# jianhengLiu/VINS-RGBD-FAST

Measured on AMD Instinct MI355X. Metric: VIO frames/sec (640x480, 150 feats, 10-KF window), higher is better.
Workload: dtype f64; 1 GPU; BASELINE configs[2]: 128 independent synthetic 640x480 RGB-D + 200 Hz IMU sequences per MI355X, 150 features, 10-keyframe window; sequences_per_gpu=128, tracker_lag=1, parallelism=sequences sharded per GPU, no data-path collective

## Files before the change

include/vio_abi.h:

```cpp
#ifndef VIO_ABI_H
#define VIO_ABI_H
#include <stddef.h>
#include <stdint.h>
#ifdef __cplusplus
extern "C" {
#endif

enum {
    VIO_OK = 0,
    VIO_NEED_IMU = 1,
    VIO_REBOOTED = 2,
    VIO_EINVAL = -1,
    VIO_EDEVICE = -2,
    VIO_ECAPACITY = -3
};

typedef struct vio_config {
    int32_t width, height;
    int32_t max_cnt, min_dist;
    int32_t grid_rows, grid_cols;
    int32_t window_size;
    int32_t max_landmarks;
    int32_t fix_depth;
    int32_t estimate_extrinsic;
// ... 121 lines not shown
int vio_get_camera(vio_batch *h, int seq, vio_camera *out);
#define VIO_SNAPSHOT_MAGIC 0x0050414E534F4956ULL
#define VIO_SNAPSHOT_FORMAT 1
typedef struct vio_snapshot_shape {
    int32_t width, height, max_cnt, min_dist, grid_rows, grid_cols, window_size, max_landmarks, fix_depth, estimate_extrinsic, estimate_td,
        max_iterations, ransac_max_iters, lk_max_level, dynamic_init, use_imu, reference_quirks, marg_exact, equalize;
    int32_t imu_capacity;
    int32_t hist_cap;
    int32_t pyramid_levels;
    int32_t reserved[2];
    double focal_length, f_threshold, depth_min, depth_max, min_parallax_px, init_depth;
} vio_snapshot_shape;
typedef struct vio_snapshot_header {
    uint64_t magic;
    uint32_t format_version;
    uint32_t abi_version;
    int64_t total_bytes;
    int64_t device_bytes;
    int64_t host_bytes;
    int64_t frames_processed;
    double last_stamp;
    int32_t tracker_lag;
    int32_t solver_flag;
    vio_snapshot_shape shape;
} vio_snapshot_header;
int vio_shape_key(const vio_config *cfg, int imu_capacity, vio_snapshot_shape *out);
int vio_snapshot_info(const void *blob, int64_t bytes, vio_snapshot_header *out);
int64_t vio_snapshot_bytes(vio_batch *h, int seq);
int vio_save_seqs(vio_batch *h, int n, const int32_t *seqs, void *dst, const int64_t *offsets, const int64_t *caps, int64_t *bytes_out);
int vio_load_seqs(vio_batch *h, int n, const int32_t *seqs, const void *src, const int64_t *offsets, const int64_t *bytes);
int64_t vio_debug_save_seq_naive(vio_batch *h, int seq, void *dst, int64_t cap);
int64_t vio_debug_snapshot_staging_bytes(vio_batch *h);
int vio_debug_snapshot_layout(vio_batch *h, int i, char *name64, int32_t *kind, int64_t *bytes_per_seq, int64_t *blob_offset);
int vio_get_tracks(vio_batch *h, int seq, int cap, int32_t *ids, int32_t *track_cnt, float *cur_pts_xy, float *cur_un_pts_xy,
                   float *pts_velocity_xy);
int vio_get_landmarks(vio_batch *h, int seq, int cap, double *out);
int vio_get_landmarks_ex(vio_batch *h, int seq, int cap, double *out12);
int vio_get_prior(vio_batch *h, int seq, double *J_nxn, double *r_n, double *x0, uint8_t *present);

int vio_get_timings(vio_batch *h, int cap, double *out_ms);
int vio_profile_begin(vio_batch *h, int max_steps);
int vio_profile_end(vio_batch *h, int cap, double *out_ms);
void *vio_get_stream(vio_batch *h);

int vio_stage_pyr_down(const uint8_t *src, int w, int h, uint8_t *dst);
int vio_stage_clahe(const uint8_t *src, int w, int h, uint8_t *dst);
int vio_stage_fast_roi(const uint8_t *img, int W, int H, int rx, int ry, int rw, int rh, int cap, float *out_xys);
int vio_lk_effective_level(int width, int height, int lk_max_level);
int vio_stage_lk(const uint8_t *prev, const uint8_t *next, int w, int h, int max_level, int n, const float *prev_pts,
                 float *next_pts_inout, uint8_t *status);
int vio_stage_ransac(const vio_config *cfg, int n, const float *p1, const float *p2, uint8_t *status);
int vio_stage_relative_r(int n, const double *corres6, double *R9);
int vio_stage_relative_r_detail(int n, const double *corres6, double *R9, int *detail8);
int vio_stage_imu_factor(const vio_config *cfg, int n, const double *dt, const double *acc, const double *gyr,
                         const double *acc0, const double *gyr0, const double *ba, const double *bg, const double *pose_i,
                         const double *sb_i, const double *pose_j, const double *sb_j, double *preint_out, double *r15,
                         double *J480);
int vio_stage_projection(const vio_config *cfg, const double *pose_i, const double *pose_j, const double *ex, double inv_dep,
                         double td, const double *obs_i, const double *obs_j, int use_td, double *r2, double *J46);
int vio_stage_projection_residual(const vio_config *cfg, const double *pose_i, const double *pose_j, const double *ex, double inv_dep,
                                  double td, const double *obs_i, const double *obs_j, int use_td, double *r2, double *J46);
int vio_stage_pnp(int n, const double *obj, const double *img, double *rvec3, double *tvec3);
int vio_stage_pnp_trace(int n, const double *obj, const double *img, double *rvec3, double *tvec3, int *trace4);
int vio_stage_host_pnp_trace(int n, const double *obj, const double *img, double *rvec3, double *tvec3, int *trace4);
int vio_stage_rodrigues(int mode, int n, const double *in, double *out);
int vio_stage_host_rodrigues(int mode, int n, const double *in, double *out);
// ... 36 lines not shown
```

vins-rgbd-fast_amd/__init__.py:

```python
import ctypes as C
import os
import subprocess

import numpy as np

_HERE = os.path.dirname(os.path.abspath(__file__))
_LIB_PATH = os.path.join(_HERE, "libvio_hip.so")

VIO_OK, VIO_NEED_IMU, VIO_REBOOTED = 0, 1, 2
VIO_EINVAL, VIO_EDEVICE, VIO_ECAPACITY = -1, -2, -3


class VioError(RuntimeError):
    pass


class Config(C.Structure):
    _fields_ = [(n, C.c_int32) for n in (
        "width", "height", "max_cnt", "min_dist", "grid_rows", "grid_cols", "window_size", "max_landmarks", "fix_depth",
        "estimate_extrinsic", "estimate_td", "max_iterations", "ransac_max_iters", "lk_max_level", "dynamic_init", "use_imu", "reference_quirks",
        "marg_exact", "equalize")] + \
        [(n, C.c_double) for n in ("fx", "fy", "cx", "cy", "k1", "k2", "p1", "p2", "focal_length", "f_threshold", "depth_min",
                                   "depth_max", "acc_n", "acc_w", "gyr_n", "gyr_w", "g_norm")] + \
        [("ric", C.c_double * 9), ("tic", C.c_double * 3)] + \
# ... 565 lines not shown
    def process_obs(self, seq, ids, obs, depth, stamp):
        ids = np.ascontiguousarray(ids, np.int32).reshape(-1)
        obs = np.ascontiguousarray(obs, np.float64).reshape(-1, 7)
        depth = np.ascontiguousarray(depth, np.uint16)
        self._keep3 = (ids, obs, depth)
        self._chk(self.L.vio_process_obs(self.h, seq, len(ids), ids.ctypes.data, obs.ctypes.data, depth.ctypes.data, float(stamp)),
                  "vio_process_obs")

    def process_obs_batch(self, n_obs, ids, obs, depth, stamps, on_device=False):
        n_obs = np.ascontiguousarray(n_obs, np.int32).reshape(self.S)
        ids = np.ascontiguousarray(ids, np.int32).reshape(self.S, -1)
        cap = ids.shape[1]
        obs = np.ascontiguousarray(obs, np.float64).reshape(self.S, cap, 7)
        stamps = np.ascontiguousarray(stamps, np.float64).reshape(self.S)
        self._keep3 = (n_obs, ids, obs, depth, stamps)
        self._chk(self.L.vio_process_obs_batch(self.h, n_obs.ctypes.data, ids.ctypes.data, obs.ctypes.data, cap, _ptr(depth),
                                               stamps.ctypes.data, 1 if on_device else 0), "vio_process_obs_batch")

    def packaged(self, seq=0, cap=2048):
        ids, obs = np.zeros(cap, np.int32), np.zeros((cap, 7))
        n = self._chk(self.L.vio_get_packaged(self.h, seq, cap, ids.ctypes.data, obs.ctypes.data), "vio_get_packaged")
        return ids[:n].copy(), obs[:n].copy()

    def solver_kind(self):
        self.L.vio_get_solver_kind.argtypes = [C.c_void_p]
        return self.L.vio_get_solver_kind(self.h)

    def bound_stats(self, seq=0):
        o = np.zeros(4, np.int64)
        self.L.vio_get_bound_stats.argtypes = [C.c_void_p, C.c_int, C.c_void_p]
        self._chk(self.L.vio_get_bound_stats(self.h, int(seq), o.ctypes.data), "vio_get_bound_stats")
        return tuple(int(x) for x in o)

    def ex_calibration(self, seq=0, history=False):
        o = np.zeros(16, np.float64)
        hist = np.zeros((2048 if history else 0, 12), np.float64)
        n = self._chk(self.L.vio_get_ex_calibration(self.h, int(seq), o.ctypes.data, hist.shape[0], hist.ctypes.data if history else None),
                      "vio_get_ex_calibration")
        out = dict(state=int(o[0]), pairs=int(o[1]), success_frame=int(o[2]), ric=o[3:12].reshape(3, 3).copy(), sv=o[12:16].copy())
        if history:
            out["history"] = hist[:min(n, hist.shape[0])].reshape(-1, 3, 4).copy()
        return out

    def marg_certificate(self, seq=0):
        o = np.zeros(2, np.int32)
        self.L.vio_get_marg_certificate.argtypes = [C.c_void_p, C.c_int, C.c_void_p]
        self._chk(self.L.vio_get_marg_certificate(self.h, int(seq), o.ctypes.data), "vio_get_marg_certificate")
        return int(o[0]), bool(o[1])

    def capacity(self):
        c = np.zeros(3, np.int32)
        self._chk(self.L.vio_get_capacity(self.h, c.ctypes.data), "vio_get_capacity")
        return dict(tracks=int(c[0]), landmarks=int(c[1]), imu=int(c[2]))

    def reset_seq(self, seq):
        self._chk(self.L.vio_reset_seq(self.h, seq), "vio_reset_seq")

    def reset_tracker_seq(self, seq):
        self._chk(self.L.vio_reset_tracker_seq(self.h, seq), "vio_reset_tracker_seq")

    def sync(self):
        self._chk(self.L.vio_sync(self.h), "vio_sync")

    def reset(self):
        self._chk(self.L.vio_reset(self.h), "vio_reset")

# ... 178 lines not shown
```

vins-rgbd-fast_amd/csrc/abi_query.hip:

```cpp
#include "vio_handle.h"

namespace vio_internal {

std::string calibration_check(const vio_calibration &k) {
    const struct { const char *name; const double *v; int n; } fin[] = {
        {"fx", &k.fx, 1}, {"fy", &k.fy, 1}, {"cx", &k.cx, 1}, {"cy", &k.cy, 1}, {"k1", &k.k1, 1}, {"k2", &k.k2, 1}, {"p1", &k.p1, 1},
        {"p2", &k.p2, 1}, {"ric", k.ric, 9}, {"tic", k.tic, 3}, {"td", &k.td, 1}, {"tr", &k.tr, 1}, {"acc_n", &k.acc_n, 1},
        {"acc_w", &k.acc_w, 1}, {"gyr_n", &k.gyr_n, 1}, {"gyr_w", &k.gyr_w, 1}, {"g_norm", &k.g_norm, 1}};
    for (const auto &f : fin)
        for (int i = 0; i < f.n; i++)
            if (!std::isfinite(f.v[i])) return std::string(f.name) + " is not finite";
    const struct { const char *name; double v; } pos[] = {
        {"fx", k.fx}, {"fy", k.fy}, {"acc_n", k.acc_n}, {"acc_w", k.acc_w}, {"gyr_n", k.gyr_n}, {"gyr_w", k.gyr_w}, {"g_norm", k.g_norm}};
    for (const auto &f : pos)
        if (!(f.v > 0)) return std::string(f.name) + " must be > 0";
    if (!(k.tr >= 0)) return "tr must be >= 0";
    {
        double err = 0;
        for (int i = 0; i < 3; i++)
            for (int j = 0; j < 3; j++) {
                double d = (i == j) ? -1.0 : 0.0;
                for (int q = 0; q < 3; q++) d += k.ric[3 * i + q] * k.ric[3 * j + q];
                err = std::max(err, std::fabs(d));
            }
// ... 433 lines not shown
    int n = h->hc.NPRIOR, W = h->hc.W;
    if (J || r) {
        be_prior_factor_kernel<<<1, 512, h->lds_factor, h->stream>>>(h->B, seq);
        HIPCHK(hipGetLastError());
        HIPCHK(hipStreamSynchronize(h->stream));
    }
    if (J) HIPCHK(hipMemcpy(J, h->B.prior_J + (size_t)seq * n * n, sizeof(double) * n * n, hipMemcpyDeviceToHost));
    if (r) HIPCHK(hipMemcpy(r, h->B.prior_rf + (size_t)seq * n, sizeof(double) * n, hipMemcpyDeviceToHost));
    if (x0) HIPCHK(hipMemcpy(x0, h->B.prior_x0 + (size_t)seq * (W * 7 + 17), sizeof(double) * (W * 7 + 17), hipMemcpyDeviceToHost));
    if (present) for (int k = 0; k < W + 3; k++) present[k] = (uint8_t)be.prior_present[k];
    return n;
}

int vio_get_timings(vio_batch *h, int cap, double *out_ms) {
    VIO_ENTER(h, VIO_NO_SEQ, false);
    if (!out_ms || cap < 3) return VIO_EINVAL;
    if (!h->timing_valid) return 0;
    VIO_TRY(sync_all(h));
    float a = 0, b = 0;
    HIPCHK(hipEventElapsedTime(&a, h->ev[0], h->ev[1]));
    HIPCHK(hipEventElapsedTime(&b, h->ev[1], h->ev[2]));
    out_ms[0] = a; out_ms[1] = b; out_ms[2] = a + b;
    return 3;
}

int vio_debug_seq(vio_batch *h, int seq, int *out16) {
    VIO_ENTER(h, seq, true);
    static thread_local BeSeq be;
    HIPCHK(hipMemcpy(&be, h->B.be + seq, sizeof(BeSeq), hipMemcpyDeviceToHost));
    for (int k = 0; k < 16; k++) out16[k] = be.dbg[k];
    return VIO_OK;
}

int vio_debug_phases(vio_batch *h, float *out128, int reset) {
    VIO_ENTER(h, VIO_NO_SEQ, true);
    if (out128) HIPCHK(hipMemcpy(out128, h->B.timings, 128 * sizeof(float), hipMemcpyDeviceToHost));
    if (reset) HIPCHK(hipMemset(h->B.timings, 0, 128 * sizeof(float)));
    return VIO_OK;
}

int vio_debug_fe_ticks(vio_batch *h, float *out) {
    VIO_ENTER(h, VIO_NO_SEQ, true);
    if (!out) return VIO_EINVAL;
    HIPCHK(hipMemcpy(out, h->B.fe_ticks, (size_t)h->S * 4 * sizeof(float), hipMemcpyDeviceToHost));
    return VIO_OK;
}

int vio_profile_begin(vio_batch *h, int max_steps) {
    VIO_ENTER(h, VIO_NO_SEQ, false);
    if (max_steps < 1) return VIO_EINVAL;
    size_t need = (size_t)max_steps * VIO_NEV;
    while (h->pev.size() < need) {
        hipEvent_t e;
        VIO_TRY(new_event(h, &e, hipEventDefault));
        h->pev.push_back(e);
    }
    h->prof_steps = max_steps;
    h->prof_cur = 0;
    h->prof_fe_only = false;
    return VIO_OK;
}
int vio_profile_end(vio_batch *h, int cap, double *out_ms) {
    VIO_ENTER(h, VIO_NO_SEQ, true);
    if (!out_ms || cap < VIO_NK) return VIO_EINVAL;
    int n = h->prof_cur < 0 ? 0 : (h->prof_cur < h->prof_steps ? h->prof_cur : h->prof_steps);
    static const int e0[VIO_NK] = {0, 1, 2, 3, 4, 5, 6, 8, 9, 10}, e1[VIO_NK] = {1, 2, 3, 4, 5, 6, 7, 9, 10, 11};
// ... 14 lines not shown
```

vins-rgbd-fast_amd/csrc/be_kernels.hip:

```cpp
#include <hip/hip_runtime.h>
#include "kernels.h"
#include "be_factors.h"

using namespace dm;

#if VIO_TIMERS
#define PH_INIT long long ph_t0 = (s == 0 && threadIdx.x == 0) ? VIO_CLOCK() : 0
#define PH(k) do { if (s == 0 && threadIdx.x == 0) { long long n_ = VIO_CLOCK(); B.timings[k] += (float)(n_ - ph_t0); ph_t0 = n_; } } while (0)
#else
#define PH_INIT do {} while (0)
#define PH(k) do {} while (0)
#endif

namespace {

struct Ctx {
    float *timings;
    const DevCfg *C;
    int s, W, P, LW, NL, NLs, NPR;
    BeSeq *be;
    FeSeq *fe;
    const vio_calibration *K;
    PreInt *pre;
    int *lm_id, *lm_start, *lm_nobs, *lm_est, *lm_solve, *lm_dyn, *lm_order, *lm_free, *lm_tmp, *lm_pidx, *lm_aidx, *lm_relo;
// ... 497 lines not shown
                } else { dep = rsum / rn; ef = 0; }
            } else { dep = vsum / vn; ef = 1; }
            if (dep < 0.1) { dep = cfg.init_depth; ef = 0; }
            c.lm_depth[slot] = dep;
            c.lm_est[slot] = ef;
        }
}

__device__ void repropagate_window(Ctx &c, PreWork &pw) {
    const int t = threadIdx.x, nt = blockDim.x, W = c.W;
    BeSeq &be = *c.be;
    const vio_config &cfg = c.C->c;
    for (int j = 0; j <= W; j++) {
            PreInt &p = c.pre[be.pre_idx[j]];
            if (!p.valid) continue;
            if (t == 0) {
                int nb = p.n_buf;
                v3 la = ld3(p.lin_acc), lg = ld3(p.lin_gyr);
                p.sum_dt = 0;
                st3(p.acc0, la); st3(p.gyr0, lg);
                p.dp[0] = p.dp[1] = p.dp[2] = 0; p.dv[0] = p.dv[1] = p.dv[2] = 0;
                p.dq[0] = 1; p.dq[1] = p.dq[2] = p.dq[3] = 0;
                p.lin_ba[0] = p.lin_ba[1] = p.lin_ba[2] = 0;
                st3(p.lin_bg, ld3(be.Bgs[j]));
                p.n_buf = nb;
            }
            for (int i = t; i < 225; i += nt) { pw.J[i] = ((i / 15) == (i % 15)) ? 1.0 : 0.0; pw.Pm[i] = 0; }
            __syncthreads();
            for (int q = 0; q < p.n_buf; q++) preint_propagate(p, pw, *c.K, p.dt_buf[q], ld3(p.acc_buf[q]), ld3(p.gyr_buf[q]));
            preint_store(p, pw);
        }
}

template <bool EXCALIB>
__global__ __launch_bounds__(256) void be_ingest_kernel(Batch B, const uint16_t *depth_base, size_t depth_stride, IngestSrc src) {
    const int s = blockIdx.x + B.s0, t = threadIdx.x, nt = blockDim.x;
    Ctx c = make_ctx(B, s);
    const DevCfg &C = *B.cfg;
    const vio_config &cfg = C.c;
    const vio_calibration &K = *c.K;
    BeSeq &be = *c.be;
    FeSeq &fe = *c.fe;
    const int W = c.W;
    __shared__ int sh_i[8];
    __shared__ double sh_d[8];
    __shared__ int scratch[2 * 256 + 8];
    __shared__ double sred[256];
    __shared__ PreWork pw;
    PH_INIT;
    const bool ext = src.ids != nullptr;
    const int ext_n = ext ? src.n_obs[s] : 0;
    const double in_stamp = ext ? src.stamps[s] : fe.cur_time;
    if (t == 0) {
        for (int k = 0; k < 3; k++) be.track_Bg[k] = be.latest_Bg[k];
        be.track_td = be.td;
        be.imu_count_ingest = be.imu_count;
        be.do_solve = 0; be.do_marg = 0; be.processed = 0; be.rebooted = 0; be.init_frame = 0; be.dyn_failed = 0;
        be.status_code = (!ext && fe.n_forw == -2) ? VIO_NEED_IMU : VIO_OK;
        be.cur_stamp = in_stamp;
        be.overflow = 0;
        if (be.imu_count - be.imu_head > C.NIMU) { be.imu_head = be.imu_count - C.NIMU; be.overflow |= 16; }
    }
    __syncthreads();
    if (ext ? ext_n <= 0 : (fe.n_forw < 0 || !fe.publish_ok)) return;
    const double *it = B.imu_t + (size_t)s * C.NIMU;
    const double *ia = B.imu_acc + (size_t)s * C.NIMU * 3, *ig = B.imu_gyr + (size_t)s * C.NIMU * 3;
    double stamp = in_stamp, curTime = stamp + be.td;
    if (cfg.use_imu) {
        bool have = be.imu_count > be.imu_head;
        double back_t = have ? it[(be.imu_count - 1) % C.NIMU] : -1e300;
        if (!(have && curTime <= back_t)) {
            if (t == 0) be.status_code = VIO_NEED_IMU;
            return;
        }
    }
    const uint16_t *depth = depth_base + (size_t)s * depth_stride;
    const int fc = be.frame_count;
    int nobs = ext ? min(ext_n, C.NP) : fe.n_obs, nlm = be.n_lm;
    const int *o_id = ext ? src.ids + (size_t)s * src.cap : B.obs_id + (size_t)s * C.NP;
    const double *o = ext ? src.obs + (size_t)s * src.cap * 7 : B.obs + (size_t)s * C.NP * 7;
    int *flag = c.lm_tmp;
    int *offs = c.lm_pidx;
    int tracked = 0;
    extern __shared__ int htab[];
    const int HT = C.lm_hash_size;
    for (int q = t; q < HT; q += nt) htab[q] = -1;
    __syncthreads();
    for (int k = t; k < nlm; k += nt) {
        int slot = c.lm_order[k], id = c.lm_id[slot];
        unsigned hsh = ((unsigned)id * 2654435761u) & (unsigned)(HT - 1);
        while (atomicCAS(&htab[hsh], -1, id) != -1) hsh = (hsh + 1) & (unsigned)(HT - 1);
        htab[HT + hsh] = slot;
    }
    __syncthreads();
    for (int j = t; j < nobs; j += nt) {
        const double *p = o + (size_t)j * 7;
        unsigned short mm = depth[(size_t)min(max((int)p[4], 0), cfg.height - 1) * cfg.width + min(max((int)p[3], 0), cfg.width - 1)];
        double dmm = mm / 1000.0;
        int isnew = 0;
        if (!(0 < dmm && dmm < cfg.depth_min)) {
            int fid = o_id[j];
            int found = -1;
            unsigned hsh = ((unsigned)fid * 2654435761u) & (unsigned)(HT - 1);
            while (htab[hsh] != -1) {
                if (htab[hsh] == fid) { found = htab[HT + hsh]; break; }
// ... 42 lines not shown
        }
        __syncthreads();
        nlm = be.n_lm;
    }
    PH(107);
    {
        double psum = 0, pnum = 0;
        if (!(fc < 2 || be.last_track_num < 20)) {
            for (int k = t; k < nlm; k += nt) {
                int slot = c.lm_order[k];
                int st = c.lm_start[slot], no = c.lm_nobs[slot];
                if (st <= fc - 2 && st + no - 1 >= fc - 1) {
                    const double *fi = obs_ptr(c, slot, fc - 2), *fj = obs_ptr(c, slot, fc - 1);
                    double dep_i = fi[2], u_i = fi[0] / dep_i, v_i = fi[1] / dep_i;
                    double du = u_i - fj[0], dv = v_i - fj[1];
                    psum += fmax(0.0, sqrt(fmin(du * du + dv * dv, du * du + dv * dv)));
                    pnum += 1.0;
                }
            }
        }
        psum = block_sum(psum, sred);
        pnum = block_sum(pnum, sred);
        if (t == 0) {
            bool kf;
            if (fc < 2 || be.last_track_num < 20) kf = true;
            else if (pnum == 0) kf = true;
            else kf = psum / pnum >= cfg.min_parallax_px / cfg.focal_length;
            be.marginalization_flag = kf ? 0 : 1;
            be.Headers[fc] = stamp;
        }
        __syncthreads();
    }
    PH(108);
    if (cfg.use_imu && t < 64) {
        const int cnt_all = be.imu_count;
        const double prevT = be.prevTime;
        int head = be.imu_head;
        for (;;) {
            const int idx = head + t;
            const bool pass = idx < cnt_all && it[idx % C.NIMU] <= prevT;
            const unsigned long long stop = ~__ballot(pass);
            if (stop) { head += __ffsll((long long)stop) - 1; break; }
            head += 64;
        }
        int k = head;
        for (;;) {
            const int idx = k + t;
            const bool pass = idx < cnt_all && it[idx % C.NIMU] < curTime;
            const unsigned long long stop = ~__ballot(pass);
            if (stop) { k += __ffsll((long long)stop) - 1; break; }
            k += 64;
        }
        sh_i[6] = head; sh_i[7] = k;
    }
    if (cfg.use_imu && t == 0) {
        const int head = sh_i[6], k = sh_i[7];
        sh_i[0] = head;
        sh_i[1] = k - head + 1;
        be.imu_head = k;
        be.n_imu_frame = sh_i[1];
        be.imu_frame_head = head;
        if (!be.initFirstPoseFlag) {
            v3 aver = mk(0, 0, 0);
            for (int q = 0; q < sh_i[1]; q++) aver = add(aver, ld3(ia + (size_t)((head + q) % C.NIMU) * 3));
            aver = scl(1.0 / (double)sh_i[1], aver);
            m3 R0 = g2R(aver);
            double yaw = R2ypr(R0).x;
            R0 = mul(ypr2R(mk(-yaw, 0, 0)), R0);
            stm(be.Rs[0], R0);
            be.initFirstPoseFlag = 1;
        }
    }
    __syncthreads();
    if (cfg.use_imu) {
        int head = sh_i[0], n = sh_i[1];
        PreInt &P = c.pre[be.pre_idx[fc]];
        if (t == 0) {
            v3 a0 = ld3(ia + (size_t)(head % C.NIMU) * 3), g0 = ld3(ig + (size_t)(head % C.NIMU) * 3);
            if (!be.first_imu) { be.first_imu = 1; st3(be.acc_0, a0); st3(be.gyr_0, g0); }
            if (!P.valid) bf::preint_init(P, ld3(be.acc_0), ld3(be.gyr_0), ld3(be.Bas[fc]), ld3(be.Bgs[fc]));
        }
        __syncthreads();
        if (fc != 0) {
            preint_load(P, pw);
            __shared__ double pi_fv[PREINT_MANY_LDS_DOUBLES];
            const PreintRing ring = {it, ia, ig, head, C.NIMU, be.prevTime, curTime, n};
            WorldStep ws = {ld3(be.acc_0), ld3(be.gyr_0), ld3(be.Ps[fc]), ld3(be.Vs[fc]), ldm(be.Rs[fc]), ld3(be.Bas[fc]), ld3(be.Bgs[fc]), ld3(be.g)};
            const int nb0 = P.n_buf;
            PH(111);
            preint_propagate_many<true>(P, pw, K, n, ring, ws, true, pi_fv);
            PH(112);
            if (t == 0 && nb0 + n > VIO_IMU_SLOT_CAP) be.overflow |= 2;
            if (t == 64) {
                stm(be.Rs[fc], ws.R); st3(be.Ps[fc], ws.P); st3(be.Vs[fc], ws.V);
                st3(be.acc_0, ws.a0); st3(be.gyr_0, ws.g0);
            }
            __syncthreads();
        } else if (t == 0) {
            const int idx = (head + n - 1) % C.NIMU;
            st3(be.acc_0, ld3(ia + (size_t)idx * 3)); st3(be.gyr_0, ld3(ig + (size_t)idx * 3));
        }
        if (fc != 0) preint_store(P, pw);
        if (t == 0) be.prevTime = curTime;
        __syncthreads();
    }
    PH(109);
    if constexpr (EXCALIB) {
// ... 2377 lines not shown
```

vins-rgbd-fast_amd/csrc/kernels.h:

```cpp
#pragma once
#include <hip/hip_runtime.h>
#include "vio_state.h"
#include "../../include/vio_synth.h"

#define PI_CH 8
#define PREINT_MANY_LDS_DOUBLES (PI_CH * (225 + 270))
__host__ __device__ static inline size_t marg_overlay_bytes(int nprior, int W, bool gj) {
    const size_t nbq = ((size_t)nprior + 15) >> 4, tiles = nbq * (nbq + 1) / 2 * 2048, t1 = (size_t)2 * nprior * 15 * 8, pi = (size_t)PREINT_MANY_LDS_DOUBLES * 8;
    size_t m = tiles > t1 ? tiles : t1;
    m = m > pi ? m : pi;
    if (gj && (size_t)W * 210 * 8 > m) m = (size_t)W * 210 * 8;
    return ((m + 15) & ~(size_t)15) + 64;
}
#define MARG_LM_TABLES 6
__host__ __device__ static inline size_t marg_resident_doubles(int nprior) { const size_t q = (size_t)nprior + 15; return q * q + q + (size_t)nprior; }
__host__ __device__ static inline size_t marg_resident_lds_bytes(int nprior, int W) { return marg_overlay_bytes(nprior, W, true) + marg_resident_doubles(nprior) * 8; }
static inline size_t fast_lds_bytes(int rw, int rh) {
    return (size_t)(((rw + 6) * rh + 15) & ~15) + (size_t)((rw * rh + 15) & ~15) + (size_t)(((rw - 6) * (rh - 6) + 63) / 64 + 2) * 8 + 16;
}
__host__ __device__ static inline size_t ps_eval_lds_bytes(int W) {
    const size_t W1 = (size_t)W + 1, a = (W1 * W1 + 1) * 32 * 8, b = (size_t)W * (VIO_PREINT_HDR + 1) * 8;
    return (a > b ? a : b) + 64;
}
static inline size_t ps_ls_lds_bytes(int W) { (void)W; return ((((sizeof(Params) / sizeof(double)) + 1) & ~(size_t)1) + 176) * 8 + 16; }
struct LkImages {
    const uint8_t *prev[4];
    const uint8_t *next[4];
    int w[4], h[4];
};

__global__ void fe_begin_kernel(Batch B, const double *stamps, int gate, int publish, const uint8_t *modes, const double *R_rel);
__global__ void be_latest_odometry_kernel(Batch B, int seq, double *out11);
__global__ void be_imu_rate_odometry_kernel(Batch B, const double *since, int cap, int *n_rows, double *rows, double *last);
__global__ void fe_predict_motion_kernel(Batch B, int seq, double t0, double t1, double *out9);
__global__ void fe_pyrdown_kernel(Batch B, const uint8_t *src_base, size_t src_stride, int sw, int sh, int dst_level, int write_level0);
__global__ void fe_pyrdown_stage_kernel(const uint8_t *src, int sw, int sh, uint8_t *dst);
__global__ void fe_clahe_lut_kernel(Batch B, const uint8_t *src_base, size_t stride);
__global__ void fe_clahe_apply_kernel(Batch B, const uint8_t *src_base, size_t stride);
__global__ void fe_clahe_lut_stage_kernel(const uint8_t *src, int W, int H, uint8_t *lut);
__global__ void fe_clahe_apply_stage_kernel(const uint8_t *src, int W, int H, const uint8_t *lut, uint8_t *dst);
__global__ void fe_predict_kernel(Batch B);
__global__ void fe_lk_kernel(Batch B);
__global__ void fe_lk_stage_kernel(LkImages im, int maxLevel, int n, const float2 *prevPts, float2 *nextPts, uint8_t *status);
__global__ void fe_ransac_stage_kernel(vio_config c, int n, const float2 *p1, const float2 *p2, uint8_t *status);
__global__ void fe_camera_stage_kernel(vio_camera cam, int n, const double *uv, const double *R9, double *ray, double *un, double *uv_out);
__global__ void fe_select_kernel(Batch B);
__global__ void fe_fast_kernel(Batch B);
__global__ void fe_fast_stage_kernel(const uint8_t *img, int W, GridRect r, uint32_t *out, int cap, int *count);
__global__ void fe_add_kernel(Batch B, int gate);
struct IngestSrc {
    const int *n_obs;
    const int *ids;
    const double *obs;
    const double *stamps;
    int cap;
};
template <bool EXCALIB> __global__ void be_ingest_kernel(Batch B, const uint16_t *depth_base, size_t depth_stride, IngestSrc src);
__global__ void be_stage_relative_r_kernel(int n, const double *corres6, double *R9, int *detail8);
__global__ void be_solve_kernel(Batch B);
__global__ void be_solve_kernel_512(Batch B);
__global__ void be_marg_kernel(Batch B);
__global__ void be_marg_hbm_kernel(Batch B);
__global__ void be_marg_exact_kernel(Batch B);
__global__ void ps_setup_kernel(Batch B);
__global__ void ps_eval_kernel(Batch B);
__global__ void ps_eval_kernel_occ3(Batch B);
__global__ void ps_eval_kernel_occ4(Batch B);
__global__ void ps_asm_a_kernel(Batch B);
__global__ void ps_asm_a_kernel_occ4(Batch B);
__global__ void ps_asm_b_schur_kernel(Batch B, int nb_b, int by_blocks);
__global__ void ps_serial_big_kernel(Batch B);
__global__ void ps_serial_kernel_512(Batch B);
__global__ void ps_final_kernel(Batch B);
__global__ void ps_ls_kernel(Batch B);
__global__ void ps_evalf_kernel(Batch B);
static inline size_t ps_evalf_lds_bytes(int W) {
    const size_t W1 = (size_t)W + 1, a = ((size_t)PS_FUSE_CAP * 28 + (W1 * W / 2 + 1) * 32) * 8 + (size_t)PS_FUSE_CAP * 12, b = ((size_t)W * (VIO_PREINT_HDR + 1) + (size_t)W * 465) * 8;
    return (a > b ? a : b) + 16;
}
__global__ void be_prior_factor_kernel(Batch B, int seq);
__global__ void be_set_relo_kernel(Batch B, int seq, const double *par);
__global__ void be_stage_pnp_kernel(const double *pts, int n, double *par6, int *trace4);
__global__ void be_stage_rodrigues_kernel(int mode, int n, const double *in, double *out);
__global__ void be_dyn_finalize_kernel(Batch B, int seq, const double *samples, const int *offs);
__global__ void be_stage_imu_kernel(vio_config cfg, PreInt *P, int n, const double *dt, const double *acc, const double *gyr,
                                    const double *par, double g_norm, double *preint_out, double *r15, double *J480);
__global__ void be_stage_projection_kernel(vio_config cfg, const double *in, int use_td, int form, double *r2, double *J46);
__global__ void be_stage_imu_block_kernel(const PreInt *P, const double *par, double g_norm, double *G961);
__global__ void be_stage_preint_kernel(vio_config cfg, PreInt *P, int n, const double *dt, const double *acc, const double *gyr, int mode,
// ... 21 lines not shown
```

vins-rgbd-fast_amd/csrc/vio_abi.hip:

```cpp
#include "vio_handle.h"

thread_local std::string g_err;

namespace {

void circle_halfwidths(int radius, int *hw) {
    for (int i = 0; i <= radius; i++) hw[i] = -1;
    int err = 0, dx = radius, dy = 0, plus = 1, minus = (radius << 1) - 1;
    while (dx >= dy) {
        if (dx > hw[dy]) hw[dy] = dx;
        if (dy > hw[dx]) hw[dx] = dy;
        dy++;
        err += plus;
        plus += 2;
        int mask = (err <= 0) - 1;
        err -= minus & mask;
        dx += mask;
        minus -= mask & 2;
    }
}

}

static size_t ingest_lds_bytes(const DevCfg &C, bool excalib) {
// ... 662 lines not shown
    h->hc.MXL = 0;
    h->hc.eig_one_wave = env_int("VIO_EIG_ONE_WAVE", 0) != 0;
    h->hc.eig_jacobi = env_int("VIO_MARG_EIG_JACOBI", 0) != 0;
    if (h->hc.MX > 0) {
        hipFuncAttributes fa;
        int cap = 0;
        if (hipDeviceGetAttribute(&cap, hipDeviceAttributeMaxSharedMemoryPerBlock, h->device) != hipSuccess || cap <= 0) cap = 160 * 1024;
        if (hipFuncGetAttributes(&fa, (const void *)be_marg_exact_kernel) == hipSuccess) {
            const long avail = (long)cap - (long)fa.sharedSizeBytes - 256;
            int m = 0;
            while (m < 128 && (long)marg_exact_lds_bytes(m + 1) <= avail) m++;
            m = std::min(m, std::max(0, env_int("VIO_MARG_EIG_LDS", m)));
            h->hc.MXL = m;
        }
    }
}

static void read_knobs(vio_batch *h) {
    h->be_threads = std::min(1024, std::max(64, env_int("VIO_BE_THREADS", h->be_threads) & ~63));
    h->asm_b_by_blocks = std::max(0, std::min(2, env_int("VIO_ASM_B_MODE", h->asm_b_by_blocks)));
    h->ps_asm_b_blocks = h->hc.W <= 10 ? 12 : 24;
    h->ps_asm_b_blocks = std::max(1, std::min(256, env_int("VIO_ASM_B_BLOCKS", h->ps_asm_b_blocks)));
    h->eval_occ = env_int("VIO_EVAL_OCC", h->eval_occ);
    h->use_graph = env_int("VIO_GRAPH", h->use_graph) != 0;
    h->xcd_map = env_int("VIO_XCD_MAP", h->xcd_map);
    h->fe_xcd_map = env_int("VIO_FE_XCD_MAP", h->fe_xcd_map);
    h->xcd_n = env_int("VIO_XCD_N", h->xcd_n);
    h->feed_throttle = env_int("VIO_FEED_THROTTLE", h->feed_throttle) != 0;
    h->uploads_in_flight = env_int("VIO_UPLOADS_IN_FLIGHT", h->uploads_in_flight) == 1 ? 1 : 2;
    h->extra_slots = std::max(1, env_int("VIO_EXTRA_SLOTS", h->extra_slots));
    h->asm_a_occ4 = env_int("VIO_ASM_A_OCC", 0) >= 4;
    h->marg_threads = std::min(512, std::max(64, env_int("VIO_MARG_THREADS", h->marg_threads) & ~63));
    h->marg_lds = env_int("VIO_MARG_LDS", 1) != 0;
    h->B.flags = env_int("VIO_FLAGS", 0);
}

static int create_groups(vio_batch *h) {
    const DevCfg &C = h->hc;
    const int n_seq = h->S;
    int per = env_int("VIO_GROUP_SEQS", n_seq);
    if (per < 1) per = 1;
    if (C.c.dynamic_init) per = n_seq;
    int ng = (n_seq + per - 1) / per;
    if (ng > 16) { ng = 16; per = (n_seq + ng - 1) / ng; ng = (n_seq + per - 1) / per; }
    h->groups.resize(ng);
    for (int k = 0; k < ng; k++) {
        vio_batch::Group &g = h->groups[k];
        g.s0 = k * per;
        g.n = std::min(per, n_seq - g.s0);
        VIO_TRY(create_group_streams(h, g, false));
        for (hipEvent_t *e : {&g.ev_solve, &g.ev_fe, &g.ev_be, &g.ev_ingest}) VIO_TRY(new_event(h, e));
    }
    h->stream = h->groups[0].stream; h->fe_stream = h->groups[0].fe_stream;
    return new_event(h, &h->ev_imu);
}

static int size_launches(vio_batch *h) {
    const DevCfg &C = h->hc;
    Batch &B = h->B;
    h->lds_select = (size_t)C.NP * 104 + 260 * 4 + 64;
    h->lds_add = (size_t)C.NP * 16 + (size_t)4 * 192 * 8  + 3 * VIO_FAST_CAP * 4 + 260 * 4 + 64 * 4 + (size_t)C.NP * 12 + 64;
    h->lds_fast = 0;
    for (int k = 0; k < C.ncells; k++) h->lds_fast = std::max(h->lds_fast, fast_lds_bytes(C.rect[k].w, C.rect[k].h));
    {
        size_t npairs = (size_t)(C.W + 1) * C.W / 2;
        size_t workd = std::max((size_t)C.W * 450, npairs * 210 <= 12288 ? npairs * 210 : (size_t)0);
// ... 77 lines not shown
    (void)raise_lds_limit(ingest, ingest_lds_bytes(C, excalib));

    (void)raise_lds_limit((const void *)fe_select_kernel, (size_t)(h->lds_select));
    (void)raise_lds_limit((const void *)fe_add_kernel, (size_t)(h->lds_add));
    (void)raise_lds_limit((const void *)fe_fast_kernel, (size_t)(h->lds_fast));
    bool fits = lds_fits(C.MX > 0 ? (const void *)be_marg_exact_kernel : h->marg_lds ? (const void *)be_marg_kernel : (const void *)be_marg_hbm_kernel, h->lds_marg, "be_marg") &&
                lds_fits(ingest, ingest_lds_bytes(C, excalib), "be_ingest") &&
                lds_fits((const void *)fe_select_kernel, h->lds_select, "fe_select") && lds_fits((const void *)fe_add_kernel, h->lds_add, "fe_add") &&
                lds_fits((const void *)fe_fast_kernel, h->lds_fast, "fe_fast");
    if (fits && h->solve_mode == 1)
        fits = lds_fits((const void *)ps_eval_kernel, h->lds_ps_eval, "ps_eval") && lds_fits((const void *)ps_ls_kernel, h->lds_ps_ls, "ps_ls") &&
               lds_fits(h->serial_big ? (const void *)ps_serial_big_kernel : (const void *)ps_serial_kernel_512, h->lds_serial, "ps_serial");
    else if (fits)
        fits = lds_fits(h->be_threads <= 512 ? (const void *)be_solve_kernel_512 : (const void *)be_solve_kernel, h->lds_solve, "be_solve");
    return fits ? VIO_OK : VIO_ECAPACITY;
}

static int handle_init(vio_batch *h, int n_seq) {
    size_marg_exact(h);
    h->S = n_seq;
    const DevCfg &C = h->hc;
    const size_t S = (size_t)n_seq, NP = C.NP;
    Batch &B = h->B;
    memset(&B, 0, sizeof(B));
    B.S = n_seq;
    B.hist_cap = 2048;
    B.s0 = 0;
    B.ns = 0; B.xcd_nb = 0; B.xcd_n = 8;
    read_knobs(h);
    VIO_TRY(handle_alloc_arrays(h));
    h->d_cal = const_cast<vio_calibration *>(B.cal);
    VIO_TRY(dev_alloc(h, &h->d_stamps, S)); VIO_TRY(dev_alloc(h, &h->d_modes, S)); VIO_TRY(dev_alloc(h, &h->d_rrel, S * 9)); VIO_TRY(dev_alloc(h, &h->d_r9, 16));
    VIO_TRY(dev_alloc(h, &h->d_in_n, S)); VIO_TRY(dev_alloc(h, &h->d_in_stamps, S)); VIO_TRY(dev_alloc(h, &h->d_in_ids, S * NP)); VIO_TRY(dev_alloc(h, &h->d_in_obs, S * NP * 7));
    B.gW = h->hc.W; B.gP = h->hc.P; B.gLW = h->hc.LW; B.gNL = h->hc.NL; B.gNP = h->hc.NP; B.gNRES = h->hc.NRES; B.gNPRIOR = h->hc.NPRIOR; B.gMX = h->hc.MX;
    HIPCHK(hipMemcpy(B.cfg, &h->hc, sizeof(DevCfg), hipMemcpyHostToDevice));
    VIO_TRY(create_groups(h));
    if (C.c.dynamic_init) {
        h->dyn.assign(n_seq, vio_batch::DynSeq());
        h->dyn_active = true;
        VIO_TRY(pinned_alloc(h, &h->h_state, S)); VIO_TRY(dev_alloc(h, &h->d_state, S, false)); VIO_TRY(new_event(h, &h->ev_state));
    }
    for (int i = 0; i < 4; i++) VIO_TRY(new_event(h, &h->ev[i], hipEventDefault));
    vio_calibration k;
    cal_from_config(C.c, k);
    h->cal.assign(n_seq, k);
    HIPCHK(hipMemcpy(h->d_cal, h->cal.data(), sizeof(vio_calibration) * n_seq, hipMemcpyHostToDevice));
    h->cam.assign(n_seq, pinhole_camera(k));
    HIPCHK(hipMemcpy(h->d_cam, h->cam.data(), sizeof(vio_camera) * n_seq, hipMemcpyHostToDevice));
    h->last_imu_t.assign(n_seq, -1e300);
    VIO_TRY(init_state(h, 0, n_seq));
    for (auto &g : h->groups) (void)hipEventRecord(g.ev_be, g.stream);
    return size_launches(h);
}

vio_batch *vio_create(const vio_config *cfg, int n_seq, int imu_capacity) { return vio_create_on_device(cfg, n_seq, imu_capacity, -1); }
int vio_get_device(vio_batch *h) { return h ? h->device : VIO_EINVAL; }

vio_batch *vio_create_on_device(const vio_config *cfg, int n_seq, int imu_capacity, int device) {
    if (!cfg || n_seq < 1) { g_err = "bad arguments"; return nullptr; }
    int ndev = 0;
    if (hipGetDeviceCount(&ndev) != hipSuccess || ndev < 1) { g_err = "no HIP device (the product path has no CPU fallback)"; return nullptr; }
    if (device >= ndev) { g_err = "vio_create_on_device: no such HIP device"; return nullptr; }
    int caller_dev = 0;
    if (hipGetDevice(&caller_dev) != hipSuccess) { g_err = "hipGetDevice failed"; return nullptr; }
    vio_batch *h = new vio_batch();
    h->device = device < 0 ? caller_dev : device;
// ... 166 lines not shown
        HIPCHK(hipMemcpyAsync(h->d_modes + g.s0, slot + n * 8, n, hipMemcpyHostToDevice, g.fe_stream));
    }
    HIPCHK(hipEventRecord(g.side_ev[k], g.fe_stream));
    g.side_used[k] = true;
    return VIO_OK;
}

static int stage_side_inputs(vio_batch *h, vio_batch::Group &g, const uint8_t *modes, const double *R_rel) {
    if (modes) HIPCHK(hipMemcpyAsync(h->d_modes + g.s0, modes + g.s0, (size_t)g.n, hipMemcpyHostToDevice, g.fe_stream));
    if (R_rel) HIPCHK(hipMemcpyAsync(h->d_rrel + (size_t)g.s0 * 9, R_rel + (size_t)g.s0 * 9, (size_t)g.n * 9 * sizeof(double), hipMemcpyHostToDevice, g.fe_stream));
    return VIO_OK;
}

int vio_feed_modes(vio_batch *h, const uint8_t *gray, const uint16_t *depth_mm, const double *stamps, const uint8_t *modes, int on_device) {
    VIO_ENTER(h, VIO_NO_SEQ, false);
    if (!gray || !depth_mm || !stamps) return VIO_EINVAL;
    VIO_TRY(wait_host_uploads(h));
    VIO_TRY(refresh_dynamic_state(h));
    VIO_TRY(flush_imu_frontend(h));
    static const bool feed_trace = env_int("VIO_FEED_TRACE", 0) != 0;
    auto now_us = []() { return std::chrono::duration<double, std::micro>(std::chrono::steady_clock::now().time_since_epoch()).count(); };
    for (auto &g : h->groups) {
        const double tt0 = feed_trace ? now_us() : 0;
        VIO_TRY(fe_wait(h, g));
        const uint8_t *dg = nullptr;
        const uint16_t *dd = nullptr;
        VIO_TRY(stage_inputs(h, g, gray, depth_mm, nullptr, on_device, &dg, &dd, true));
        const double tt1 = feed_trace ? now_us() : 0;
        VIO_TRY(stage_side_ring(h, g, stamps, modes));
        if (g.s0 == 0) HIPCHK(hipEventRecord(h->ev[0], g.fe_stream));
        VIO_TRY(launch_frontend(h, g, dg, 1, 1, modes ? h->d_modes : nullptr, nullptr));
        if (g.s0 == 0) HIPCHK(hipEventRecord(h->ev[1], g.fe_stream));
        if (!on_device) VIO_TRY(note_stage_read(h, g.ev_rd_gray[g.flip], g.have_rd_gray[g.flip], g.fe_stream));
        VIO_TRY(be_wait(g));
        VIO_TRY(launch_backend(h, g, dd, kTrackerMap));
        if (!on_device) {
            VIO_TRY(note_stage_read(h, g.ev_rd_depth[g.flip], g.have_rd_depth[g.flip], g.stream));
            g.flip ^= 1;
        }
        if (g.s0 == 0) HIPCHK(hipEventRecord(h->ev[2], g.stream));
        if (feed_trace) fprintf(stderr, "vio_feed group %d: stage_inputs %.0f us, rest (side ring + %s launches) %.0f us, t = %.0f\n", g.s0, tt1 - tt0, "all", now_us() - tt1, tt0);
    }
    if (h->prof_cur >= 0) h->prof_cur++;
    h->timing_valid = true;
    return VIO_OK;
}

int vio_abi_version(void) { return 12; }
int vio_abi_sizeof(int what) {
    return what == 0 ? (int)sizeof(vio_config) : what == 1 ? (int)sizeof(vio_status) : what == 2 ? (int)sizeof(vio_calibration)
         : what == 3 ? (int)sizeof(vio_camera) : what == 4 ? (int)sizeof(vio_snapshot_header) : what == 5 ? (int)sizeof(vio_snapshot_shape) : -1;
}

int vio_host_buffers_done(vio_batch *h, int calls_ago) {
    VIO_ENTER(h, VIO_NO_SEQ, false);
    if (calls_ago < 0) return VIO_EINVAL;
    if (calls_ago > 1) return 1;
    for (auto &g : h->groups) {
        if (!g.copy_stream) continue;
        const int p = (g.flip ^ 1 ^ calls_ago) & 1;
        if (!g.up_used[p]) continue;
        for (hipEvent_t e : {g.ev_up_gray[p], g.ev_up_depth[p]}) {
            const hipError_t q = hipEventQuery(e);
            if (q == hipErrorNotReady) return 0;
            if (q != hipSuccess) { g_err = "hipEventQuery failed"; return VIO_EDEVICE; }
        }
    }
    return 1;
// ... 188 lines not shown
```

vins-rgbd-fast_amd/csrc/vio_handle.h:

```cpp
#pragma once
#include <hip/hip_runtime.h>
#include <limits.h>
#include <math.h>
#include <algorithm>
#include <cmath>
#include <stdlib.h>
#include <mutex>
#include <chrono>
#include <string>
#include <string.h>
#include <vector>
#include "kernels.h"
#include "dyninit_host.h"
#include "camera_model.h"
#include "snapshot.h"
#include "stage_util.h"

struct vio_batch {
    DevCfg hc;
    Batch B;
    int S;
    int device = -1;
    struct Group {
        int s0 = 0, n = 0;
// ... 56 lines not shown
        bool nonlinear = false;
        int attempts = 0, failures = 0, last_stage = 0;
    };
    std::vector<DynSeq> dyn;
    bool dyn_active = false;
    int *h_state = nullptr;
    int *d_state = nullptr;
    hipEvent_t ev_state = nullptr;
    bool state_pending = false;
    double *d_dyn_samples = nullptr;
    int *d_dyn_offs = nullptr;
    size_t dyn_samples_cap = 0;
    std::mutex imu_mu;
    std::vector<int> p_seq;
    std::vector<double> p_t, p_acc, p_gyr;
    struct ImuStage {
        int *h_seq = nullptr, *d_seq = nullptr;
        double *h_t = nullptr, *h_acc = nullptr, *h_gyr = nullptr, *d_t = nullptr, *d_acc = nullptr, *d_gyr = nullptr;
        size_t cap = 0;
        hipEvent_t done = nullptr;
        bool busy = false;
    } imu_stage[2];
    int imu_stage_cur = 0;
    hipEvent_t ev_imu = nullptr;
    std::vector<double> last_imu_t;
    size_t lds_select = 0, lds_add = 0, lds_fast = 0, lds_solve = 0, lds_serial = 0, lds_marg = 0, lds_factor = 0, lds_ps_ls = 0, lds_ps_evalf = 0;
    int ps_evalf_blocks = 0;
    bool feed_throttle = true;
    int uploads_in_flight = 2;
    int relo_frames = 0;
    bool line_search = true;
    int be_threads = 512, marg_threads = 384;
    bool marg_lds = true;
    int solve_mode = 1;
    bool asm_a_occ4 = false;
    int eval_occ = 0;
    bool serial_big = false;
    size_t lds_ps_eval = 0;
    int ps_eval_blocks = 0, ps_asm_a_blocks = 0, ps_schur_tiles = 0;
    bool timing_valid = false;
    std::vector<hipEvent_t> pev;
    int prof_steps = 0, prof_cur = -1;
    bool prof_fe_only = false;
    struct SnapRow { const char *name; int kind; unsigned char *base; int64_t bytes, blob_off; };
    std::vector<SnapRow> snap_rows;
    int64_t snap_dev_bytes = 0, snap_chunks = 0;
    int snap_entries = 0;
    SnapEntry *d_snap_tab = nullptr;
    SnapSeq *d_snap_seqs = nullptr;
    size_t snap_seqs_cap = 0;
    unsigned char *d_snap_stage = nullptr;
    size_t snap_stage_cap = 0;
};
#define VIO_NK 10
#define VIO_NEV 12
#define PEV(h, k) do { if (g.s0 == 0 && (h)->prof_cur >= 0 && (h)->prof_cur < (h)->prof_steps) (void)hipEventRecord((h)->pev[(size_t)(h)->prof_cur * VIO_NEV + (k)], (k) <= 7 ? g.fe_stream : g.stream); } while (0)

inline int env_int(const char *name, int dflt) {
    const char *v = getenv(name);
    return v ? atoi(v) : dflt;
}

inline int raise_lds_limit(const void *fn, size_t bytes) {
    struct Seen { const void *fn; int dev; size_t bytes; };
    static std::mutex mu;
    static std::vector<Seen> seen;
// ... 217 lines not shown
```

Baseline: 61280 frames/s.

## Precompute IMU preintegration ahead on frontend stream and adopt it in ingest

Adds a kernel that runs IMU preintegration for the upcoming frame on the frontend stream once the previous solve has finished, storing the result with a snapshot of its inputs. The backend ingest kernel compares those inputs bit-for-bit and, when they match, copies the precomputed preintegration and world-state instead of integrating itself. The aim is to take IMU propagation off the serial backend critical path by overlapping it with frontend work. In exchange it adds a per-frame kernel launch, a cross-stream wait on the solve event when tracker lag is on, a validation pass, and a large per-sequence record copy. The fallback to in-kernel integration is kept whenever the check fails.

```diff
diff --git a/include/vio_abi.h b/include/vio_abi.h
--- a/include/vio_abi.h
+++ b/include/vio_abi.h
@@ -177,6 +177,7 @@
 int64_t vio_debug_save_seq_naive(vio_batch *h, int seq, void *dst, int64_t cap);
 int64_t vio_debug_snapshot_staging_bytes(vio_batch *h);
 int vio_debug_snapshot_layout(vio_batch *h, int i, char *name64, int32_t *kind, int64_t *bytes_per_seq, int64_t *blob_offset);
+int vio_debug_preint_ahead(vio_batch *h, int64_t *out2, int64_t *per_seq);
 int vio_get_tracks(vio_batch *h, int seq, int cap, int32_t *ids, int32_t *track_cnt, float *cur_pts_xy, float *cur_un_pts_xy,
                    float *pts_velocity_xy);
 int vio_get_landmarks(vio_batch *h, int seq, int cap, double *out);
diff --git a/vins-rgbd-fast_amd/__init__.py b/vins-rgbd-fast_amd/__init__.py
--- a/vins-rgbd-fast_amd/__init__.py
+++ b/vins-rgbd-fast_amd/__init__.py
@@ -621,6 +621,12 @@
         self._chk(self.L.vio_get_bound_stats(self.h, int(seq), o.ctypes.data), "vio_get_bound_stats")
         return tuple(int(x) for x in o)
 
+    def preint_ahead_stats(self, per_seq=False):
+        o, ps = np.zeros(2, np.int64), np.zeros((self.S, 2), np.int64)
+        self.L.vio_debug_preint_ahead.argtypes = [C.c_void_p, C.c_void_p, C.c_void_p]
+        self._chk(self.L.vio_debug_preint_ahead(self.h, o.ctypes.data, ps.ctypes.data), "vio_debug_preint_ahead")
+        return ps if per_seq else (int(o[0]), int(o[1]))
+
     def ex_calibration(self, seq=0, history=False):
         o = np.zeros(16, np.float64)
         hist = np.zeros((2048 if history else 0, 12), np.float64)
diff --git a/vins-rgbd-fast_amd/csrc/abi_query.hip b/vins-rgbd-fast_amd/csrc/abi_query.hip
--- a/vins-rgbd-fast_amd/csrc/abi_query.hip
+++ b/vins-rgbd-fast_amd/csrc/abi_query.hip
@@ -489,6 +489,23 @@
     return VIO_OK;
 }
 
+int vio_debug_preint_ahead(vio_batch *h, int64_t *out2, int64_t *per_seq) {
+    VIO_ENTER(h, VIO_NO_SEQ, true);
+    if (!out2) return VIO_EINVAL;
+    out2[0] = out2[1] = 0;
+    if (per_seq) memset(per_seq, 0, (size_t)h->S * 2 * sizeof(int64_t));
+    if (!h->d_ahead) return VIO_OK;
+    const size_t head = offsetof(PreAhead, pre);
+    std::vector<unsigned char> rec(head);
+    for (int s = 0; s < h->S; s++) {
+        HIPCHK(hipMemcpy(rec.data(), h->d_ahead + s, head, hipMemcpyDeviceToHost));
+        const PreAhead *r = (const PreAhead *)rec.data();
+        out2[0] += (int64_t)r->used; out2[1] += (int64_t)r->declined;
+        if (per_seq) { per_seq[2 * s] = (int64_t)r->used; per_seq[2 * s + 1] = (int64_t)r->declined; }
+    }
+    return VIO_OK;
+}
+
 int vio_debug_phases(vio_batch *h, float *out128, int reset) {
     VIO_ENTER(h, VIO_NO_SEQ, true);
     if (out128) HIPCHK(hipMemcpy(out128, h->B.timings, 128 * sizeof(float), hipMemcpyDeviceToHost));
diff --git a/vins-rgbd-fast_amd/csrc/be_kernels.hip b/vins-rgbd-fast_amd/csrc/be_kernels.hip
--- a/vins-rgbd-fast_amd/csrc/be_kernels.hip
+++ b/vins-rgbd-fast_amd/csrc/be_kernels.hip
@@ -553,6 +553,126 @@
         }
 }
 
+__device__ __forceinline__ void imu_interval_search(const double *it, int NIMU, int cnt_all, double prevT, double curTime, int head0, int &head, int &k) {
+    const int t = threadIdx.x & 63;
+    head = head0;
+    for (;;) {
+        const int idx = head + t;
+        const bool pass = idx < cnt_all && it[idx % NIMU] <= prevT;
+        const unsigned long long stop = ~__ballot(pass);
+        if (stop) { head += __ffsll((long long)stop) - 1; break; }
+        head += 64;
+    }
+    k = head;
+    for (;;) {
+        const int idx = k + t;
+        const bool pass = idx < cnt_all && it[idx % NIMU] < curTime;
+        const unsigned long long stop = ~__ballot(pass);
+        if (stop) { k += __ffsll((long long)stop) - 1; break; }
+        k += 64;
+    }
+}
+__device__ __forceinline__ const double *ahead_in_ptr(const BeSeq &be, int W, int i) {
+    return i < 3 ? be.acc_0 + i : i < 6 ? be.gyr_0 + (i - 3) : i < 9 ? be.Ps[W] + (i - 6) : i < 12 ? be.Vs[W] + (i - 9) : i < 21 ? be.Rs[W] + (i - 12)
+         : i < 24 ? be.Bas[W] + (i - 21) : i < 27 ? be.Bgs[W] + (i - 24) : be.g + (i - 27);
+}
+__device__ __forceinline__ bool same_bits(double a, double b) { return __double_as_longlong(a) == __double_as_longlong(b); }
+
+__global__ __launch_bounds__(256) void be_preint_ahead_kernel(Batch B, const double *stamps, PreAhead *ahead) {
+    const int s = blockIdx.x + B.s0, t = threadIdx.x;
+    Ctx c = make_ctx(B, s);
+    const DevCfg &C = *B.cfg;
+    const vio_calibration &K = *c.K;
+    const BeSeq &be = *c.be;
+    const int W = c.W;
+    PreAhead &rec = ahead[s];
+    __shared__ int sh_i[8];
+    __shared__ double sh_in[30];
+    __shared__ PreWork pw;
+    __shared__ double pi_fv[PREINT_MANY_LDS_DOUBLES];
+    const double *it = B.imu_t + (size_t)s * C.NIMU;
+    const double *ia = B.imu_acc + (size_t)s * C.NIMU * 3, *ig = B.imu_gyr + (size_t)s * C.NIMU * 3;
+    const double stamp = stamps[s], prevT = be.prevTime, curTime = stamp + be.td;
+    const int head0 = be.imu_head, cnt_all = be.imu_count;
+    if (t < 30) sh_in[t] = *ahead_in_ptr(be, W, t);
+    if (t == 0) {
+        bool ok = C.c.use_imu && W > 0 && be.solver_flag == 1 && be.frame_count == W && !be.rebooted && be.first_imu && be.initFirstPoseFlag;
+        ok = ok && head0 >= 0 && cnt_all > head0 && cnt_all - head0 <= C.NIMU;
+        ok = ok && curTime <= it[(cnt_all - 1) % C.NIMU];
+        sh_i[0] = ok;
+        if (!ok) rec.valid = 0;
+    }
+    __syncthreads();
+    if (!sh_i[0]) return;
+    if (t < 64) {
+        int head, k;
+        imu_interval_search(it, C.NIMU, cnt_all, prevT, curTime, head0, head, k);
+        sh_i[6] = head; sh_i[7] = k;
+    }
+    PreInt &P = rec.pre;
+    if (t == 0) {
+        rec.valid = 0;
+        rec.stamp = stamp; rec.cur_time = curTime; rec.prev_time = prevT;
+        rec.imu_head = head0; rec.imu_count = cnt_all;
+        rec.noise[0] = K.acc_n; rec.noise[1] = K.gyr_n; rec.noise[2] = K.acc_w; rec.noise[3] = K.gyr_w;
+        bf::preint_init(P, ld3(sh_in), ld3(sh_in + 3), ld3(sh_in + 21), ld3(sh_in + 24));
+    }
+    if (t >= 64 && t < 94) rec.in[t - 64] = sh_in[t - 64];
+    __syncthreads();
+    const int head = sh_i[6], n = sh_i[7] - head + 1;
+    preint_load(P, pw);
+    const PreintRing ring = {it, ia, ig, head, C.NIMU, prevT, curTime, n};
+    WorldStep ws = {ld3(sh_in), ld3(sh_in + 3), ld3(sh_in + 6), ld3(sh_in + 9), ldm(sh_in + 12), ld3(sh_in + 21), ld3(sh_in + 24), ld3(sh_in + 27)};
+    preint_propagate_many<true>(P, pw, K, n, ring, ws, true, pi_fv);
+    if (t == 64) { st3(rec.out, ws.P); st3(rec.out + 3, ws.V); stm(rec.out + 6, ws.R); st3(rec.out + 15, ws.a0); st3(rec.out + 18, ws.g0); }
+    preint_store(P, pw);
+    if (t == 0) { rec.head = head; rec.k = sh_i[7]; rec.n = n; rec.valid = 1; }
+}
+
+__device__ __forceinline__ bool preint_ahead_take(Ctx &c, PreAhead &rec, double stamp, double curTime, int *sh_flag) {
+    const int t = threadIdx.x, nt = blockDim.x, W = c.W;
+    BeSeq &be = *c.be;
+    const vio_calibration &K = *c.K;
+    PreInt &P = c.pre[be.pre_idx[W]];
+    if (t < 64) {
+        bool ok = true;
+        if (t < 30) ok = same_bits(rec.in[t], *ahead_in_ptr(be, W, t));
+        else if (t < 42) { const int i = t - 30; ok = same_bits(P.lin_acc[i], rec.in[i < 6 ? i : i + 15]); }
+        else if (t == 42) ok = same_bits(rec.noise[0], K.acc_n) && same_bits(rec.noise[1], K.gyr_n) && same_bits(rec.noise[2], K.acc_w) && same_bits(rec.noise[3], K.gyr_w);
+        else if (t == 43) ok = same_bits(rec.stamp, stamp) && same_bits(rec.cur_time, curTime) && same_bits(rec.prev_time, be.prevTime);
+        else if (t == 44) ok = rec.valid == 1 && rec.imu_head == be.imu_head && rec.imu_count == be.imu_count && P.valid && P.n_buf == 0 && be.first_imu && be.initFirstPoseFlag;
+        const bool all = __ballot(ok) == ~0ull;
+        if (t == 0) *sh_flag = all;
+    }
+    __syncthreads();
+    if (!*sh_flag) return false;
+    const int n = rec.n, m = min(n, VIO_IMU_SLOT_CAP);
+    const PreInt &Q = rec.pre;
+    {
+        double *d = (double *)&P;
+        const double *q = (const double *)&Q;
+        for (int i = t; i < (int)(offsetof(PreInt, dt_buf) / sizeof(double)); i += nt) d[i] = q[i];
+        for (int i = t; i < m; i += nt) P.dt_buf[i] = Q.dt_buf[i];
+        for (int i = t; i < 3 * m; i += nt) { (&P.acc_buf[0][0])[i] = (&Q.acc_buf[0][0])[i]; (&P.gyr_buf[0][0])[i] = (&Q.gyr_buf[0][0])[i]; }
+    }
+    if (t >= 64 && t < 85) {
+        const int i = t - 64;
+        double *d = i < 3 ? be.Ps[W] + i : i < 6 ? be.Vs[W] + (i - 3) : i < 15 ? be.Rs[W] + (i - 6) : i < 18 ? be.acc_0 + (i - 15) : be.gyr_0 + (i - 18);
+        *d = rec.out[i];
+    }
+    if (t == 0) {
+        P.n_buf = Q.n_buf;
+        be.imu_head = rec.k;
+        be.n_imu_frame = n;
+        be.imu_frame_head = rec.head;
+        be.prevTime = curTime;
+        if (n > VIO_IMU_SLOT_CAP) be.overflow |= 2;
+        rec.used++;
+    }
+    __syncthreads();
+    return true;
+}
+
 template <bool EXCALIB>
 __global__ __launch_bounds__(256) void be_ingest_kernel(Batch B, const uint16_t *depth_base, size_t depth_stride, IngestSrc src) {
     const int s = blockIdx.x + B.s0, t = threadIdx.x, nt = blockDim.x;
@@ -583,7 +703,11 @@
         if (be.imu_count - be.imu_head > C.NIMU) { be.imu_head = be.imu_count - C.NIMU; be.overflow |= 16; }
     }
     __syncthreads();
-    if (ext ? ext_n <= 0 : (fe.n_forw < 0 || !fe.publish_ok)) return;
+    PreAhead *const ahead = src.ahead ? src.ahead + s : nullptr;
+    if (ext ? ext_n <= 0 : (fe.n_forw < 0 || !fe.publish_ok)) {
+        if (ahead && t == 0) ahead->declined++;
+        return;
+    }
     const double *it = B.imu_t + (size_t)s * C.NIMU;
     const double *ia = B.imu_acc + (size_t)s * C.NIMU * 3, *ig = B.imu_gyr + (size_t)s * C.NIMU * 3;
     double stamp = in_stamp, curTime = stamp + be.td;
@@ -591,7 +715,7 @@
         bool have = be.imu_count > be.imu_head;
         double back_t = have ? it[(be.imu_count - 1) % C.NIMU] : -1e300;
         if (!(have && curTime <= back_t)) {
-            if (t == 0) be.status_code = VIO_NEED_IMU;
+            if (t == 0) { be.status_code = VIO_NEED_IMU; if (ahead) ahead->declined++; }
             return;
         }
     }
@@ -700,28 +824,17 @@
         __syncthreads();
     }
     PH(108);
-    if (cfg.use_imu && t < 64) {
-        const int cnt_all = be.imu_count;
-        const double prevT = be.prevTime;
-        int head = be.imu_head;
-        for (;;) {
-            const int idx = head + t;
-            const bool pass = idx < cnt_all && it[idx % C.NIMU] <= prevT;
-            const unsigned long long stop = ~__ballot(pass);
-            if (stop) { head += __ffsll((long long)stop) - 1; break; }
-            head += 64;
-        }
-        int k = head;
-        for (;;) {
-            const int idx = k + t;
-            const bool pass = idx < cnt_all && it[idx % C.NIMU] < curTime;
-            const unsigned long long stop = ~__ballot(pass);
-            if (stop) { k += __ffsll((long long)stop) - 1; break; }
-            k += 64;
-        }
+    bool imu_here = cfg.use_imu;
+    if (ahead && imu_here) {
+        if (fc == W && fc != 0 && preint_ahead_take(c, *ahead, stamp, curTime, &sh_i[5])) imu_here = false;
+        else if (t == 0) ahead->declined++;
+    }
+    if (imu_here && t < 64) {
+        int head, k;
+        imu_interval_search(it, C.NIMU, be.imu_count, be.prevTime, curTime, be.imu_head, head, k);
         sh_i[6] = head; sh_i[7] = k;
     }
-    if (cfg.use_imu && t == 0) {
+    if (imu_here && t == 0) {
         const int head = sh_i[6], k = sh_i[7];
         sh_i[0] = head;
         sh_i[1] = k - head + 1;
@@ -740,7 +853,7 @@
         }
     }
     __syncthreads();
-    if (cfg.use_imu) {
+    if (imu_here) {
         int head = sh_i[0], n = sh_i[1];
         PreInt &P = c.pre[be.pre_idx[fc]];
         if (t == 0) {
diff --git a/vins-rgbd-fast_amd/csrc/kernels.h b/vins-rgbd-fast_amd/csrc/kernels.h
--- a/vins-rgbd-fast_amd/csrc/kernels.h
+++ b/vins-rgbd-fast_amd/csrc/kernels.h
@@ -48,13 +48,27 @@
 __global__ void fe_fast_kernel(Batch B);
 __global__ void fe_fast_stage_kernel(const uint8_t *img, int W, GridRect r, uint32_t *out, int cap, int *count);
 __global__ void fe_add_kernel(Batch B, int gate);
+struct PreAhead;
 struct IngestSrc {
     const int *n_obs;
     const int *ids;
     const double *obs;
     const double *stamps;
     int cap;
+    PreAhead *ahead;
 };
+struct PreAhead {
+    double stamp, cur_time, prev_time;
+    double in[30], noise[4];
+    int imu_head, imu_count;
+    int valid;
+    int head, k, n;
+    double out[21];
+    unsigned long long used, declined;
+    PreInt pre;
+};
+static_assert(offsetof(PreInt, dt_buf) == (VIO_PREINT_HDR + 225) * sizeof(double), "PreInt: what be_ingest takes over from a PreAhead whole");
+__global__ void be_preint_ahead_kernel(Batch B, const double *stamps, PreAhead *ahead);
 template <bool EXCALIB> __global__ void be_ingest_kernel(Batch B, const uint16_t *depth_base, size_t depth_stride, IngestSrc src);
 __global__ void be_stage_relative_r_kernel(int n, const double *corres6, double *R9, int *detail8);
 __global__ void be_solve_kernel(Batch B);
diff --git a/vins-rgbd-fast_amd/csrc/vio_abi.hip b/vins-rgbd-fast_amd/csrc/vio_abi.hip
--- a/vins-rgbd-fast_amd/csrc/vio_abi.hip
+++ b/vins-rgbd-fast_amd/csrc/vio_abi.hip
@@ -718,6 +718,7 @@
     h->asm_a_occ4 = env_int("VIO_ASM_A_OCC", 0) >= 4;
     h->marg_threads = std::min(512, std::max(64, env_int("VIO_MARG_THREADS", h->marg_threads) & ~63));
     h->marg_lds = env_int("VIO_MARG_LDS", 1) != 0;
+    h->preint_ahead = env_int("VIO_PREINT_AHEAD", 1) != 0;
     h->B.flags = env_int("VIO_FLAGS", 0);
 }
 
@@ -861,6 +862,7 @@
     h->d_cal = const_cast<vio_calibration *>(B.cal);
     VIO_TRY(dev_alloc(h, &h->d_stamps, S)); VIO_TRY(dev_alloc(h, &h->d_modes, S)); VIO_TRY(dev_alloc(h, &h->d_rrel, S * 9)); VIO_TRY(dev_alloc(h, &h->d_r9, 16));
     VIO_TRY(dev_alloc(h, &h->d_in_n, S)); VIO_TRY(dev_alloc(h, &h->d_in_stamps, S)); VIO_TRY(dev_alloc(h, &h->d_in_ids, S * NP)); VIO_TRY(dev_alloc(h, &h->d_in_obs, S * NP * 7));
+    if (h->preint_ahead && C.c.use_imu) VIO_TRY(dev_alloc(h, &h->d_ahead, S));
     B.gW = h->hc.W; B.gP = h->hc.P; B.gLW = h->hc.LW; B.gNL = h->hc.NL; B.gNP = h->hc.NP; B.gNRES = h->hc.NRES; B.gNPRIOR = h->hc.NPRIOR; B.gMX = h->hc.MX;
     HIPCHK(hipMemcpy(B.cfg, &h->hc, sizeof(DevCfg), hipMemcpyHostToDevice));
     VIO_TRY(create_groups(h));
@@ -1093,8 +1095,16 @@
         VIO_TRY(launch_frontend(h, g, dg, 1, 1, modes ? h->d_modes : nullptr, nullptr));
         if (g.s0 == 0) HIPCHK(hipEventRecord(h->ev[1], g.fe_stream));
         if (!on_device) VIO_TRY(note_stage_read(h, g.ev_rd_gray[g.flip], g.have_rd_gray[g.flip], g.fe_stream));
+        IngestSrc src = kTrackerMap;
+        if (h->d_ahead && g.have_solve_ev) {
+            if (h->tracker_lag) HIPCHK(hipStreamWaitEvent(g.fe_stream, g.ev_solve, 0));
+            Batch Bg = h->B;
+            Bg.s0 = g.s0;
+            be_preint_ahead_kernel<<<g.n, 256, 0, g.fe_stream>>>(Bg, h->d_stamps, h->d_ahead);
+            src.ahead = h->d_ahead;
+        }
         VIO_TRY(be_wait(g));
-        VIO_TRY(launch_backend(h, g, dd, kTrackerMap));
+        VIO_TRY(launch_backend(h, g, dd, src));
         if (!on_device) {
             VIO_TRY(note_stage_read(h, g.ev_rd_depth[g.flip], g.have_rd_depth[g.flip], g.stream));
             g.flip ^= 1;
diff --git a/vins-rgbd-fast_amd/csrc/vio_handle.h b/vins-rgbd-fast_amd/csrc/vio_handle.h
--- a/vins-rgbd-fast_amd/csrc/vio_handle.h
+++ b/vins-rgbd-fast_amd/csrc/vio_handle.h
@@ -112,6 +112,8 @@
     bool line_search = true;
     int be_threads = 512, marg_threads = 384;
     bool marg_lds = true;
+    bool preint_ahead = true;
+    PreAhead *d_ahead = nullptr;
     int solve_mode = 1;
     bool asm_a_occ4 = false;
     int eval_occ = 0;
```

Result: faster. 62400 frames/s, median of 6 (+1.8%).
